# warlock-labs/sylow

Hardware: AMD Instinct MI355X
Metric: BN254 pairings/s (value) and BLS verifies/s (config.bls_verifies_per_s) at batch=2^20 per GPU (higher is better)
Workload: dtype i32/u32 limbs (9x29-bit carry-free core + 8x32-bit Montgomery, exact integer)

## Files before the change

sylow_amd/csrc/bn254_pair29.hpp:

```cpp
#pragma once
#include "bn254_f29.hpp"
#include "bn254_pair.hpp"

namespace bn254 {
namespace pl {

struct W2 { F29 c; };
BN_DEV const F29& f29_of(const W2& a) { return a.c; }
BN_DEV F29& f29_of(W2& a) { return a.c; }
struct W6 { W2 c0, c1, c2; };
struct W12 { W6 c0, c1; };

BN_DEV F29 xchg9(const F29& a) {
  F29 r;
#pragma unroll
  for (int i = 0; i < 9; ++i) r.v[i] = (i32)swap_u32((u32)a.v[i]);
  return r;
}
BN_DEV F29 sel9(bool odd, const F29& if_even, const F29& if_odd) {
  F29 r;
#pragma unroll
  for (int i = 0; i < 9; ++i) r.v[i] = odd ? if_odd.v[i] : if_even.v[i];
  return r;
}
// ... 174 lines not shown
  r.c1.c1 = w2_xi_lin(t2.v2, 1, w2_sub(w2_sub(t2.y1, t0.c1), t1.c1), 1);
  r.c1.c2 = w2_lin2(w2_sub(t2.y2, t0.c2), 1, t1.c2, -1);
}
BN_DEV W12 w12_mul(const W12& a, const W12& b) {
  const W6 t0 = w6_mul(a.c0, b.c0);
  const W6 t1 = w6_mul(a.c1, b.c1);
  const W6Raw t2 = w6_mul_raw(w6_add_norm(a.c0, a.c1), w6_add_norm(b.c0, b.c1));
  W12 r;
  w12_mul_c1(r, t2, t0, t1);
  r.c0.c0 = w2_xi_lin(t1.c2, 1, t0.c0, 1);
  r.c0.c1 = w2_norm(w2_add(t0.c1, t1.c0));
  r.c0.c2 = w2_norm(w2_add(t0.c2, t1.c1));
  return r;
}
BN_DEV W6 w6_mul_b2zero(const W6& a, const W6& b) {
  W2 v0, v1, p21, p20;
  W2_MUL2(v0, v1, a.c0, b.c0, a.c1, b.c1);
  W2_MUL2(p21, p20, a.c2, b.c1, a.c2, b.c0);
  const W2 s1 = w2_mul(w2_sub(a.c0, a.c1), w2_sub(b.c0, b.c1));
  W6 r;
  r.c0 = w2_xi_lin(p21, 1, v0, 1);
  r.c1 = w2_reduce(w2_sub(w2_add(v0, v1), s1));
  r.c2 = w2_norm(w2_add(p20, v1));
  return r;
}
BN_DEV W12 w12_mul_line_pair(const W12& a, const W12& b) {
  const W6 t0 = w6_mul(a.c0, b.c0);
  const W6 t1 = w6_mul_b2zero(a.c1, b.c1);
  const W6Raw t2 = w6_mul_raw(w6_add_norm(a.c0, a.c1), W6{w2_norm(w2_add(b.c0.c0, b.c1.c0)), w2_norm(w2_add(b.c0.c1, b.c1.c1)), b.c0.c2});
  W12 r;
  w12_mul_c1(r, t2, t0, t1);
  r.c0.c0 = w2_xi_lin(t1.c2, 1, t0.c0, 1);
  r.c0.c1 = w2_norm(w2_add(t0.c1, t1.c0));
  r.c0.c2 = w2_norm(w2_add(t0.c2, t1.c1));
  return r;
}
template <bool INL = false>
BN_DEV W12 w12_sqr(const W12& a) {
  const W6 d{w2_norm(w2_sub(a.c0.c0, a.c1.c0)), w2_norm(w2_sub(a.c0.c1, a.c1.c1)), w2_norm(w2_sub(a.c0.c2, a.c1.c2))};
  W6 e;
  e.c0 = w2_xi_lin(a.c1.c2, -1, a.c0.c0, 1);
  e.c1 = w2_norm(w2_sub(a.c0.c1, a.c1.c0));
  e.c2 = w2_norm(w2_sub(a.c0.c2, a.c1.c1));
  const W6 c2 = w6_mul<INL>(a.c0, a.c1);
  const W6Raw m = w6_mul_raw<INL>(d, e);
  W12 r;
  r.c1.c0 = w2_norm(w2_add(c2.c0, c2.c0));
  r.c1.c1 = w2_norm(w2_add(c2.c1, c2.c1));
  r.c1.c2 = w2_norm(w2_add(c2.c2, c2.c2));
  r.c0.c0 = w2_xi_lin(w2_add(m.x0, c2.c2), 1, w2_add(m.v0, c2.c0), 1);
  {
    const F29 xo = xchg9(m.v2.c);
    const W2 cc = w2_add(c2.c1, c2.c0);
    const F29* const t[4] = {&m.v2.c, &xo, &m.y1.c, &cc.c};
    const i32 c[4] = {bn_keep(9), bn_keep_v(lane_odd() ? 1 : -1), bn_keep(1), bn_keep(1)};
    r.c0.c1 = W2{f29_reduce_terms(t, c)};
  }
  r.c0.c2 = w2_lin2(m.y2, 1, w2_add(c2.c2, c2.c1), 1);
  return r;
}
BN_DEV W12 w12_conj(const W12& a) {
  W12 r;
  r.c0 = a.c0;
  r.c1.c0 = w2_norm(w2_neg(a.c1.c0)); r.c1.c1 = w2_norm(w2_neg(a.c1.c1)); r.c1.c2 = w2_norm(w2_neg(a.c1.c2));
  return r;
}
BN_DEV W2 w2_conj(const W2& a) { return W2{sel9(lane_odd(), a.c, f29_norm(f29_neg(a.c)))}; }
template <int E>
BN_DEV W6 w6_frobenius(const W6& a) {
  constexpr bool oddE = (E & 1) != 0;
  const uint32_t (&k1)[2][8] = (E == 1) ? C_FROB6_C1_1 : (E == 2) ? C_FROB6_C1_2 : C_FROB6_C1_3;
  const uint32_t (&k2)[2][8] = (E == 1) ? C_FROB6_C2_1 : (E == 2) ? C_FROB6_C2_2 : C_FROB6_C2_3;
  W6 r;
  r.c0 = oddE ? w2_conj(a.c0) : a.c0;
  W2_MUL2(r.c1, r.c2, oddE ? w2_conj(a.c1) : a.c1, w2_const(k1), oddE ? w2_conj(a.c2) : a.c2, w2_const(k2));
  return r;
}
template <int E>
BN_DEV W12 w12_frobenius(const W12& a) {
  const uint32_t (&k)[2][8] = (E == 1) ? C_FROB12_C1_1 : (E == 2) ? C_FROB12_C1_2 : C_FROB12_C1_3;
  const W2 kk = w2_const(k);
  const W6 x1 = w6_frobenius<E>(a.c1);
  W6 y;
  W2_MUL2(y.c0, y.c1, x1.c0, kk, x1.c1, kk);
  y.c2 = w2_mul(x1.c2, kk);
  return W12{w6_frobenius<E>(a.c0), y};
}
BN_DEV W12 w12_sparse_mul(const W12& f, const W2& x0, const W2& x4, const W2& x2) {
  const W2 z0 = f.c0.c0, z1 = f.c0.c1, z2 = f.c0.c2, z3 = f.c1.c0, z4 = f.c1.c1, z5 = f.c1.c2;
  W2 d0, d2, d4, p12, p54, p10, p34, p30, p52, q02, q24, q04;
  W2_MUL2(d0, d2, z0, x0, z2, x2);
  W2_MUL2(d4, p12, z4, x4, z1, x2);
  W2_MUL2(p54, p10, z5, x4, z1, x0);
  W2_MUL2(p34, p30, z3, x4, z3, x0);
  W2_MUL2(p52, q02, z5, x2, w2_sub(z0, z2), w2_sub(x0, x2));
  W2_MUL2(q24, q04, w2_sub(z2, z4), w2_sub(x2, x4), w2_sub(z0, z4), w2_sub(x0, x4));
  const W2 qs = w2_mul(w2_norm(w2_add(w2_add(z1, z3), z5)), w2_norm(w2_add(w2_add(x0, x2), x4)));
  W12 o;
  o.c0.c0 = w2_xi_lin(w2_add(p12, d4), 1, d0, 1);
  o.c0.c1 = w2_xi_lin(w2_add(p54, d2), 1, p10, 1);
  o.c0.c2 = w2_reduce(w2_add(w2_sub(w2_add(d0, d2), q02), p34));
  o.c1.c0 = w2_xi_lin(w2_sub(w2_add(d2, d4), q24), 1, p30, 1);
  o.c1.c1 = w2_xi_lin(p52, 1, w2_sub(w2_add(d0, d4), q04), 1);
  {
    const W2 sa = w2_add(w2_add(p12, p54), p10), sb = w2_add(w2_add(p34, p30), p52);
    const F29* const t[3] = {&qs.c, &sa.c, &sb.c};
    const i32 c[3] = {bn_keep(1), bn_keep(-1), bn_keep(-1)};
    o.c1.c2 = W2{f29_reduce_terms(t, c)};
  }
  return o;
}
BN_DEV W2 w2_xi_lin_v(const W2& x, const W2& y, i32 m) {
  const F29 xo = xchg9(x.c);
  const F29* const t[3] = {&x.c, &xo, &y.c};
  const i32 c[3] = {bn_keep(9), bn_keep_v(lane_odd() ? 1 : -1), bn_keep_v(m)};
  return W2{f29_reduce_terms(t, c)};
}
BN_DEV W2 w2_lin_v(const W2& x, const W2& y, i32 m) {
  const F29* const t[2] = {&x.c, &y.c};
  const i32 c[2] = {bn_keep(1), bn_keep_v(m)};
  return W2{f29_reduce_terms(t, c)};
}
BN_DEV W12 w12_sparse_mul_unit(const W12& f, i32 u, const W2& x4, const W2& x2) {
  const W2 z0 = f.c0.c0, z1 = f.c0.c1, z2 = f.c0.c2, z3 = f.c1.c0, z4 = f.c1.c1, z5 = f.c1.c2;
  W2 d2, d4, p12, p54, p34, p52, a02, a04, q24, q13;
  W2_MUL2(d2, d4, z2, x2, z4, x4);
  W2_MUL2(p12, p54, z1, x2, z5, x4);
  W2_MUL2(p34, p52, z3, x4, z5, x2);
  W2_MUL2(a02, a04, z0, x2, z0, x4);
  const W2 x24 = w2_sub(x2, x4);
  W2_MUL2(q24, q13, w2_sub(z2, z4), x24, w2_sub(z1, z3), x24);
  W12 o;
  o.c0.c0 = w2_xi_lin_v(w2_add(p12, d4), z0, u);
  o.c0.c1 = w2_xi_lin_v(w2_add(p54, d2), z1, u);
  o.c0.c2 = w2_lin_v(w2_add(a02, p34), z2, u);
  o.c1.c0 = w2_xi_lin_v(w2_sub(w2_add(d2, d4), q24), z3, u);
  {
    const F29 xo = xchg9(p52.c);
    const F29* const t[4] = {&p52.c, &xo, &a04.c, &z4.c};
    const i32 c[4] = {bn_keep(9), bn_keep_v(lane_odd() ? 1 : -1), bn_keep(1), bn_keep_v(u)};
    o.c1.c1 = W2{f29_reduce_terms(t, c)};
  }
  o.c1.c2 = w2_lin_v(w2_sub(w2_add(p12, p34), q13), z5, u);
  return o;
}
BN_DEV W2 w2_xi_norm(const W2& x, const W2& y) {
  const F29 xo = xchg9(x.c);
  const F29* const t[3] = {&x.c, &xo, &y.c};
  const i32 c[3] = {bn_keep(9), bn_keep_v(lane_odd() ? 1 : -1), bn_keep(1)};
  return W2{f29_norm_terms(t, c)};
}
BN_DEV W2 w2_xi_norm_sub(const W2& x, const W2& y) {
  const F29 xo = xchg9(x.c);
  const F29* const t[3] = {&x.c, &xo, &y.c};
  const i32 c[3] = {bn_keep(-9), bn_keep_v(lane_odd() ? -1 : 1), bn_keep(1)};
  return W2{f29_norm_terms(t, c)};
}
template <bool INL = false>
BN_DEV void w_fp4_square_fold(W2& out0, W2& m, const W2& a, const W2& b, const W2& z) {
  W2 w;
  W2_MUL2_SEL(INL, m, w, a, b, w2_sub(a, b), w2_xi_norm_sub(b, a));
  const F29 mo = xchg9(m.c);
  const F29* const t[4] = {&w.c, &m.c, &mo, &z.c};
  const i32 c[4] = {bn_keep(3), bn_keep(30), bn_keep_v(lane_odd() ? 3 : -3), bn_keep(-2)};
  out0 = W2{f29_reduce_terms(t, c)};
}
template <bool INL = false>
BN_DEV W12 w12_cyclotomic_sqr(const W12& f) {
  const W2 z0 = f.c0.c0, z4 = f.c0.c1, z3 = f.c0.c2, z2 = f.c1.c0, z1 = f.c1.c1, z5 = f.c1.c2;
  W2 m;
  W12 r;
  w_fp4_square_fold<INL>(r.c0.c0, m, z0, z1, z0);
  r.c1.c1 = w2_lin2(m, 6, z1, 2);
  w_fp4_square_fold<INL>(r.c0.c1, m, z2, z3, z4);
  r.c1.c2 = w2_lin2(m, 6, z5, 2);
  w_fp4_square_fold<INL>(r.c0.c2, m, z4, z5, z3);
  r.c1.c0 = w2_xi_lin(m, 6, z2, 2);
  return r;
}

BN_DEV F29 f29_halve(const F29& a) {
  i32 p[9]; f29_p(p);
  const i32 m = -(a.v[0] & 1);
  i32 lo[9];
  i32 c = 0;
#pragma unroll
  for (int i = 0; i < 8; ++i) {
    i32 t = a.v[i] + (p[i] & m) + c;
    lo[i] = t & BN_M29;
    c = t >> 29;
  }
  lo[8] = a.v[8] + (p[8] & m) + c;
  F29 r;
#pragma unroll
  for (int i = 0; i < 8; ++i) r.v[i] = (lo[i] >> 1) | ((lo[i + 1] & 1) << 28);
  r.v[8] = lo[8] >> 1;
  return r;
}
BN_DEV W2 w2_halve(const W2& a) { return W2{f29_halve(a.c)}; }
BN_DEV W2 w2_triple(const W2& a) { return W2{f29_add(f29_add(a.c, a.c), a.c)}; }
struct G2W { W2 x, y, z; };
BN_DEV W2 w2_twist_b() {
  const F29 k0{{0x12cb9911, 0x1fcb719e, 0x1368f727, 0x1ff96726, 0x0aadc75b, 0x179b4484, 0x06475c9b, 0x020e578d, -1520355}};
  const F29 k1{{0x0322ef99, 0x06e86c1b, 0x13f74e78, 0x0a0a4222, 0x0bcef269, 0x0af6e9ff, 0x0644c3a7, 0x0acd7c01, -535829}};
  return W2{sel9(lane_odd(), k0, k1)};
}
BN_DEV F29 f29_iso_s2() { return F29{{0x05beeef0, 0x1f76bf90, 0x1d5e46cf, 0x17f6764e, 0x1df385e5, 0x0d7a8334, 0x152215eb, 0x01b6eac1, -290196}}; }
BN_DEV F29 f29_iso_s3() { return F29{{0x1af1f8a3, 0x00cd9858, 0x1dce6a34, 0x142e620a, 0x1bc0c667, 0x0ae94d20, 0x0db9310b, 0x12572b72, 0x000405e6}}; }
BN_DEV W2 w2_mul_27m3u(const W2& a) {
  const F29 ao = xchg9(a.c);
  const F29* const t[2] = {&a.c, &ao};
  const i32 c[2] = {bn_keep(27), bn_keep_v(lane_odd() ? -3 : 3)};
  return W2{f29_reduce_terms(t, c)};
}
template <bool ISO = false>
BN_DEV void g2_doubling_step29(G2W& r, W2& l0, W2& l1, W2& l2) {
#if BN_QUAD
  W2 xy, xx, b, c, yz2, e;
  W2_MUL_SQR(xy, xx, r.x, r.y, r.x);
  const W2 a = w2_halve(xy);
  l2 = w2_norm(w2_triple(xx));
  W2_SQR2(b, c, r.y, r.z);
  if (ISO) {
    yz2 = w2_sqr(w2_norm(w2_add(r.y, r.z)));
    e = w2_mul_27m3u(c);
  } else {
    W2_SQR_MUL(yz2, e, w2_norm(w2_add(r.y, r.z)), w2_twist_b(), w2_norm(w2_triple(c)));
  }
  const W2 h = w2_norm(w2_sub(yz2, w2_add(b, c)));
  l1 = w2_neg(h);
  l0 = w2_xi_lin(w2_sub(e, b), 1, b, 0);
  const W2 f = w2_norm(w2_triple(e));
  W2_MUL2(r.z, r.x, b, h, a, w2_sub(b, f));
  const W2 g = w2_halve(w2_norm(w2_add(b, f)));
  W2 gg, ee;
  W2_SQR2(gg, ee, g, e);
  r.y = w2_lin2(gg, 1, ee, -3);
#else
  const W2 a = w2_halve(w2_mul(r.x, r.y));
  l2 = w2_norm(w2_triple(w2_sqr(r.x)));
  const W2 b = w2_sqr(r.y);
  const W2 c = w2_sqr(r.z);
  const W2 h = w2_norm(w2_sub(w2_sqr(w2_norm(w2_add(r.y, r.z))), w2_add(b, c)));
  const W2 e = ISO ? w2_mul_27m3u(c) : w2_mul(w2_twist_b(), w2_norm(w2_triple(c)));
  l1 = w2_neg(h);
  r.z = w2_mul(b, h);
  l0 = w2_xi_lin(w2_sub(e, b), 1, b, 0);
  const W2 f = w2_norm(w2_triple(e));
  r.x = w2_mul(a, w2_sub(b, f));
  const W2 g = w2_halve(w2_norm(w2_add(b, f)));
  r.y = w2_lin2(w2_sqr(g), 1, w2_sqr(e), -3);
#endif
}
BN_DEV void g2_addition_step29(G2W& r, const W2& bx, const W2& by, W2& l0, W2& l1, W2& l2) {
#if BN_QUAD
  W2 zbx, zby, ebx, dby;
  W2_MUL2(zbx, zby, r.z, bx, r.z, by);
  const W2 d = w2_sub(r.x, zbx);
  const W2 e = w2_sub(r.y, zby);
  W2_MUL2(ebx, dby, e, bx, d, by);
  l0 = w2_xi_lin(w2_sub(ebx, dby), 1, bx, 0);
  l1 = d;
  l2 = w2_neg(e);
  const W2 dn = w2_norm(d), en = w2_norm(e);
  W2 f, ee, h, i, zee, zh, dj, hy;
  W2_SQR2(f, ee, dn, en);
  W2_MUL2(h, i, dn, f, r.x, f);
  W2_MUL2(zee, zh, r.z, ee, r.z, h);
  const W2 j = w2_norm(w2_sub(w2_add(zee, h), w2_add(i, i)));
  W2_MUL2(dj, hy, dn, j, h, r.y);
  r.z = zh;
  r.x = dj;
  r.y = w2_norm(w2_sub(w2_mul(en, w2_sub(i, j)), hy));
#else
  const W2 d = w2_sub(r.x, w2_mul(r.z, bx));
  const W2 e = w2_sub(r.y, w2_mul(r.z, by));
  l0 = w2_xi_lin(w2_sub(w2_mul(e, bx), w2_mul(d, by)), 1, bx, 0);
  l1 = d;
  l2 = w2_neg(e);
  const W2 dn = w2_norm(d), en = w2_norm(e);
  const W2 f = w2_sqr(dn);
  const W2 h = w2_mul(dn, f);
  const W2 i = w2_mul(r.x, f);
  const W2 j = w2_norm(w2_sub(w2_add(w2_mul(r.z, w2_sqr(en)), h), w2_add(i, i)));
  r.z = w2_mul(r.z, h);
  r.x = w2_mul(dn, j);
  r.y = w2_norm(w2_sub(w2_mul(en, w2_sub(i, j)), w2_mul(h, r.y)));
#endif
}
BN_DEV W12 w12_line_product(const W2& a0, const W2& a4, const W2& a2, const W2& b0, const W2& b4, const W2& b2) {
  W2 d0, d2, d4, k02, k24, k04;
  W2_MUL2(d0, d2, a0, b0, a2, b2);
  W2_MUL2(d4, k02, a4, b4, w2_sub(a0, a2), w2_sub(b0, b2));
  W2_MUL2(k24, k04, w2_sub(a2, a4), w2_sub(b2, b4), w2_sub(a0, a4), w2_sub(b0, b4));
  W12 r;
  r.c0.c0 = w2_xi_lin(d4, 1, d0, 1);
  r.c0.c1 = w2_xi_lin(d2, 1, d2, 0);
  r.c0.c2 = w2_reduce(w2_sub(w2_add(d0, d2), k02));
  r.c1.c0 = w2_xi_lin(w2_sub(w2_add(d2, d4), k24), 1, d2, 0);
  r.c1.c1 = w2_reduce(w2_sub(w2_add(d0, d4), k04));
  r.c1.c2 = W2{F29{{0, 0, 0, 0, 0, 0, 0, 0, 0}}};
  return r;
}
constexpr int MILLER_LDS_WORDS = 36, MILLER_LDS_WORDS_PARK = 63;
BN_DEV void lds_put9(i32 (*lds)[256], int slot, const F29& a) {
#pragma unroll
  for (int i = 0; i < 9; ++i) lds[9 * slot + i][threadIdx.x] = a.v[i];
}
BN_DEV F29 lds_get9(i32 (*lds)[256], int slot) {
  F29 r;
#pragma unroll
  for (int i = 0; i < 9; ++i) r.v[i] = lds[9 * slot + i][threadIdx.x];
  return r;
}
#ifndef BN_MILLER_SQR_INL
#define BN_MILLER_SQR_INL false
#endif
template <bool PARK, bool ISO = false>
BN_NOINLINE void miller_loop29g(S12& fout, const Fp& pxs, const Fp& pys, const S2& qxs_in, const S2& qys_in) {
  __shared__ i32 lds[PARK ? MILLER_LDS_WORDS_PARK : MILLER_LDS_WORDS][256];
  S2 qxs = qxs_in, qys = qys_in;
  {
    const F29 px = f29_reduce(f29_from_fp(pxs)), py = f29_reduce(f29_from_fp(pys));
    lds_put9(lds, 0, ISO ? f29_mul(px, f29_iso_s2()) : px);
    lds_put9(lds, 1, ISO ? f29_mul(py, f29_iso_s3()) : py);
  }
  {
    W2 qx = w2_from_s2(qxs), qy = w2_from_s2(qys);
    if (ISO) {
      W2_SCALE2(qx, qy, qx, f29_iso_s2(), qy, f29_iso_s3());
      qxs = w2_to_s2(qx); qys = w2_to_s2(qy);
    }
    lds_put9(lds, 2, qx.c);
    lds_put9(lds, 3, qy.c);
  }
  auto PX = [&]() { return lds_get9(lds, 0); };
  auto PY = [&]() { return lds_get9(lds, 1); };
  auto QX = [&]() { return W2{lds_get9(lds, 2)}; };
  auto QY = [&](bool neg) { const W2 y{lds_get9(lds, 3)}; return neg ? w2_neg(y) : y; };
  auto park = [&](const G2W& r) { if (PARK) { lds_put9(lds, 4, r.x.c); lds_put9(lds, 5, r.y.c); lds_put9(lds, 6, r.z.c); } };
  auto unpark = [&](const G2W& r) { return PARK ? G2W{W2{lds_get9(lds, 4)}, W2{lds_get9(lds, 5)}, W2{lds_get9(lds, 6)}} : r; };
  W12 f;
  G2W r{QX(), QY(false), w2_from_s2(s2_one())};
  W2 l0, l1, l2;
  auto line_mul = [&](const W12& x) {
    W2 s1, s2;
    W2_SCALE2(s1, s2, l1, PY(), l2, PX());
    return w12_sparse_mul(x, l0, s1, s2);
  };
  const u64 nz = BN_ATE_NAF_NZ, ng = BN_ATE_NAF_NEG;
  static_assert((BN_ATE_NAF_NZ >> 63) & 1, "the first digit of 6x+2 after the leading one is non-zero");
  {
    g2_doubling_step29<ISO>(r, l0, l1, l2);
    const W2 d0 = l0;
    W2 d4, d2, e4, e2;
    W2_SCALE2(d4, d2, l1, PY(), l2, PX());
    g2_addition_step29(r, QX(), QY((ng >> 63) & 1), l0, l1, l2);
    park(r);
    W2_SCALE2(e4, e2, l1, PY(), l2, PX());
    f = w12_line_product(d0, d4, d2, l0, e4, e2);
  }
#pragma unroll 1
  for (int i = 1; i < 64; ++i) {
    r = unpark(r);
    g2_doubling_step29<ISO>(r, l0, l1, l2);
    park(r);
    f = w12_sqr<BN_MILLER_SQR_INL>(f);
    f = line_mul(f);
    if ((nz >> (63 - i)) & 1) {
      r = unpark(r);
      g2_addition_step29(r, QX(), QY((ng >> (63 - i)) & 1), l0, l1, l2);
      park(r);
      f = line_mul(f);
    }
  }
  r = unpark(r);
  S2 q1x, q1y, q2x, q2y;
  g2_psi_affine(q1x, q1y, qxs, qys);
  g2_psi_affine(q2x, q2y, q1x, q1y);
  q2y = s2_neg(q2y);
  g2_addition_step29(r, w2_from_s2(q1x), w2_from_s2(q1y), l0, l1, l2);
  f = line_mul(f);
  g2_addition_step29(r, w2_from_s2(q2x), w2_from_s2(q2y), l0, l1, l2);
  f = line_mul(f);
  w12_to_s12(fout, f);
}


BN_DEV void w12_pin(W12& x) {
  W2* const c[6] = {&x.c0.c0, &x.c0.c1, &x.c0.c2, &x.c1.c0, &x.c1.c1, &x.c1.c2};
#pragma unroll
  for (int j = 0; j < 6; ++j)
#pragma unroll
    for (int i = 0; i < 9; ++i) BN_CHAIN_NV(c[j]->c.v[i]);
}
BN_NOINLINE void w12_mul_nl(W12& r, const W12& a, const W12& b) {
  W12 x = a, y = b;
  w12_pin(x); w12_pin(y);
  r = w12_mul(x, y);
}
BN_NOINLINE void w12_cyclotomic_sqr_nl(W12& r, const W12& a) {
  W12 x = a;
  w12_pin(x);
  r = w12_cyclotomic_sqr(x);
}
template <int E> BN_NOINLINE void w12_frobenius_nl(W12& r, const W12& a) {
  W12 x = a;
  w12_pin(x);
  r = w12_frobenius<E>(x);
}
#ifndef BN_EXP_INL
#define BN_EXP_INL true
#endif
#define BN_X_C_NZ 0x0008144402208421ull
#define BN_X_C_NEG 0x0008004400000020ull
#define BN_X_C_17 0x0000100000008021ull
BN_NOINLINE void exp_by_neg_z29(W12& r, const W12& f) {
  W12 tab[2];
  {
    W12 t, u;
    w12_cyclotomic_sqr_nl(t, f);
    w12_cyclotomic_sqr_nl(u, t);
    w12_cyclotomic_sqr_nl(t, u);
    w12_cyclotomic_sqr_nl(u, t);
    w12_mul_nl(tab[0], u, f);
    w12_cyclotomic_sqr_nl(t, tab[0]);
    w12_mul_nl(tab[1], t, f);
  }
  W12 res = tab[1];
  const u64 nz = BN_X_C_NZ, ng = BN_X_C_NEG, i17 = BN_X_C_17;
#pragma unroll 1
  for (int i = 56; i >= 0; --i) {
    res = w12_cyclotomic_sqr<BN_EXP_INL>(res);
    if ((nz >> i) & 1) {
      W12 m = tab[((i17 >> i) & 1) ? 0 : 1];
      if ((ng >> i) & 1) m = w12_conj(m);
      res = w12_mul(res, m);
    }
  }
  r = w12_conj(res);
}
BN_DEV W2 w2_inv(const W2& a) {
  const F29 t = f29_mul_leaf(W_ARGS(a.c), W_ARGS(a.c));
  const F29 n = f29_norm(f29_add(t, xchg9(t)));
  const F29 i = f29_reduce(f29_from_fp(fp_inv(f29_to_fp(n))));
  const F29 r = f29_mul_leaf(W_ARGS(a.c), W_ARGS(i));
  return W2{sel9(lane_odd(), r, f29_norm(f29_neg(r)))};
}
BN_DEV W2 w2_mul_xi(const W2& a) { return w2_xi_lin(a, 1, a, 0); }
BN_DEV W6 w6_inv(const W6& a) {
  W2 s0, m12, s2, m01, s1, m02, u1, u2, o0, o1;
  W2_SQR_MUL(s0, m12, a.c0, a.c1, w2_mul_xi(a.c2));
  W2_SQR_MUL(s2, m01, a.c2, a.c0, a.c1);
  W2_SQR_MUL(s1, m02, a.c1, a.c0, a.c2);
  const W2 t0 = w2_sub(s0, m12);
  const W2 t1 = w2_sub(w2_mul_xi(s2), m01);
  const W2 t2 = w2_sub(s1, m02);
  W2_MUL2(u1, u2, a.c2, t1, a.c1, t2);
  const W2 d = w2_xi_lin(w2_add(u1, u2), 1, w2_mul(a.c0, t0), 1);
  const W2 di = w2_inv(d);
  W2_MUL2(o0, o1, di, t0, di, t1);
  return W6{o0, o1, w2_mul(di, t2)};
}
BN_NOINLINE void w12_inv_nl(W12& r, const W12& ain) {
  W12 a = ain;
  w12_pin(a);
  const W6 s0 = w6_mul(a.c0, a.c0), s1 = w6_mul(a.c1, a.c1);
  const W6 d{w2_norm(w2_sub(s0.c0, w2_mul_xi(s1.c2))), w2_norm(w2_sub(s0.c1, s1.c0)), w2_norm(w2_sub(s0.c2, s1.c1))};
  const W6 t = w6_inv(d);
  r.c0 = w6_mul(a.c0, t);
  const W6 m = w6_mul(a.c1, t);
  r.c1 = W6{w2_norm(w2_neg(m.c0)), w2_norm(w2_neg(m.c1)), w2_norm(w2_neg(m.c2))};
}
BN_NOINLINE void final_exponentiation29(S12& out, const S12& fin) {
  W12 in, t, a, b, d, e, g;
  {
    w12_from_s12(t, fin);
    w12_inv_nl(b, t);
    a = w12_conj(t);
    w12_mul_nl(d, a, b);
    w12_frobenius_nl<2>(a, d);
    w12_mul_nl(in, a, d);
  }
  exp_by_neg_z29(a, in);
  w12_cyclotomic_sqr_nl(b, a);
  w12_cyclotomic_sqr_nl(t, b);
  w12_mul_nl(d, t, b);
  exp_by_neg_z29(e, d);
  w12_cyclotomic_sqr_nl(t, e);
  exp_by_neg_z29(g, t);
  d = w12_conj(d);
  g = w12_conj(g);
  w12_mul_nl(t, g, e);
  w12_mul_nl(a, t, d);
  w12_mul_nl(d, a, b);
  w12_mul_nl(t, a, e);
  w12_mul_nl(e, in, t);
  w12_frobenius_nl<1>(t, d);
  w12_mul_nl(b, t, e);
  w12_frobenius_nl<2>(t, a);
  w12_mul_nl(e, t, b);
  t = w12_conj(in);
  w12_mul_nl(a, t, d);
  w12_frobenius_nl<3>(t, a);
  w12_mul_nl(g, t, e);
  w12_to_s12(out, g);
}


#ifdef BN_WIDE_LEAF_CALL
BN_DEV W2 w2_mul_w(const W2& a, const W2& b) { return w2_mul(a, b); }
#else
BN_DEV W2 w2_mul_w(const W2& a, const W2& b) { return w2_mul_inl(a, b); }
#endif
struct alignas(16) WideLds { i32 v[63][2][12]; };
typedef __attribute__((address_space(3))) WideLds* WideLdsPtr;
template <int EPW> BN_DEV int wide_j(int lane) { return (int)pair_index((u32)lane) & (32 / EPW - 1); }
typedef i32 __attribute__((ext_vector_type(4))) WideVec4;
typedef __attribute__((address_space(3))) WideVec4* WideVec4Ptr;
BN_DEV void wide_put(WideLdsPtr x, int slot, int odd, const W2& a) {
  const WideVec4Ptr p = (WideVec4Ptr)&x->v[slot][odd][0];
  p[0] = WideVec4{a.c.v[0], a.c.v[1], a.c.v[2], a.c.v[3]};
  p[1] = WideVec4{a.c.v[4], a.c.v[5], a.c.v[6], a.c.v[7]};
  x->v[slot][odd][8] = a.c.v[8];
}
BN_DEV W2 wide_get(WideLdsPtr x, int slot, int odd) {
  const WideVec4Ptr p = (WideVec4Ptr)&x->v[slot][odd][0];
  const WideVec4 lo = p[0], hi = p[1];
  W2 r;
  r.c.v[0] = lo.x; r.c.v[1] = lo.y; r.c.v[2] = lo.z; r.c.v[3] = lo.w;
  r.c.v[4] = hi.x; r.c.v[5] = hi.y; r.c.v[6] = hi.z; r.c.v[7] = hi.w;
  r.c.v[8] = x->v[slot][odd][8];
  return r;
}
BN_DEV W2 w2_pick(const W2& a, const W2& b, bool c) { return W2{sel9(c, a.c, b.c)}; }
BN_DEV W2 w2_real(const F29& k) { return W2{sel9(lane_odd(), k, F29{{0, 0, 0, 0, 0, 0, 0, 0, 0}})}; }
BN_DEV W2 w2_sel3(int k, const W2& a, const W2& b, const W2& c) { return w2_pick(w2_pick(a, b, k == 1), c, k == 2); }
template <int EPW = 1>
BN_DEV W12 w12_cyclotomic_sqr_wide(const W12& f, WideLdsPtr x) {
  const int lane = (int)(threadIdx.x & 63u), odd = pair_role((u32)lane), j = wide_j<EPW>(lane);
  const int p = j < 6 ? j : 0, k = p >> 1;
  const bool s = (p & 1) != 0;
  const W2 z0 = f.c0.c0, z4 = f.c0.c1, z3 = f.c0.c2, z2 = f.c1.c0, z1 = f.c1.c1, z5 = f.c1.c2;
  const W2 a = w2_sel3(k, z0, z2, z4), b = w2_sel3(k, z1, z3, z5);
  {
    const W2 xs = w2_pick(a, w2_norm(w2_add(a, b)), s), ys = w2_pick(b, w2_xi_norm(b, a), s);
    const W2 pr = w2_mul_w(xs, ys);
    if (j < 6) wide_put(x, p, odd, pr);
  }
  __syncthreads();
  {
    const int ko = p < 2 ? 0 : p < 4 ? 2 : 1;
    const bool ta = p == 0 || p == 3 || p == 4, tc = p == 2;
    const W2 m = wide_get(x, 2 * ko, odd), w = wide_get(x, 2 * ko + 1, odd);
    const W2 z = w2_pick(a, b, s);
    const F29 mo = xchg9(m.c);
    const bool lo = lane_odd();
    const F29* const t[4] = {&w.c, &m.c, &mo, &z.c};
    const i32 c[4] = {bn_keep_v(ta ? 3 : 0), bn_keep_v(ta ? -30 : tc ? 54 : 6), bn_keep_v(ta ? (lo ? -3 : 3) : tc ? (lo ? 6 : -6) : 0), bn_keep_v(ta ? -2 : 2)};
    const W2 r{f29_reduce_terms(t, c)};
    if (j < 6) wide_put(x, 6 + (p < 2 ? p : p < 4 ? p + 2 : p - 2), odd, r);
  }
  __syncthreads();
  W12 r;
  r.c0.c0 = wide_get(x, 6, odd); r.c1.c1 = wide_get(x, 7, odd); r.c0.c1 = wide_get(x, 8, odd);
  r.c1.c2 = wide_get(x, 9, odd); r.c1.c0 = wide_get(x, 10, odd); r.c0.c2 = wide_get(x, 11, odd);
  return r;
}
constexpr int WL_IA = 12, WL_IB = 18, WL_SA = 24, WL_SB = 27, WL_P = 30, WL_T = 48, WL_OUT = 57;
constexpr int WK_DENSE = 0, WK_LINE = 1, WK_SQUARE = 2;
#ifndef BN_WIDE_MILLER_INL
#define BN_WIDE_MILLER_INL 2
#endif
#ifndef BN_WIDE_KINDS
#define BN_WIDE_KINDS 1
#endif
BN_DEV W2 w12_coef(const W12& a, int c) {
  const W2 lo = w2_sel3(c % 3, a.c0.c0, a.c0.c1, a.c0.c2), hi = w2_sel3(c % 3, a.c1.c0, a.c1.c1, a.c1.c2);
  return w2_pick(lo, hi, c >= 3);
}
template <int EPW = 1, int KIND = WK_DENSE>
BN_DEV void w12_mul_wide_stage0(const W12& a, const W12& b, WideLdsPtr x) {
  const int lane = (int)(threadIdx.x & 63u), odd = pair_role((u32)lane), j = wide_j<EPW>(lane);
  {
    const int c = j < 6 ? j : 0;
    const int i = c % 3;
    const W2 a0i = w2_sel3(i, a.c0.c0, a.c0.c1, a.c0.c2), a1i = w2_sel3(i, a.c1.c0, a.c1.c1, a.c1.c2);
    const W2 sa = w2_norm(w2_add(a0i, a1i));
    if (KIND == WK_SQUARE) {
      const W2 sb0 = w2_xi_lin(a.c1.c2, 1, a.c0.c0, 1);
      const W2 sb12 = w2_norm(w2_add(a0i, w2_pick(a.c1.c0, a.c1.c1, i == 2)));
      if (j < 3) { wide_put(x, WL_IA + i, odd, a0i); wide_put(x, WL_IB + i, odd, a1i); wide_put(x, WL_SA + i, odd, sa); }
      if (j >= 3 && j < 6) wide_put(x, WL_SB + i, odd, w2_pick(sb12, sb0, i == 0));
    } else {
      const W2 ac = w2_pick(a0i, a1i, c >= 3), bc = w12_coef(b, c);
      const W2 sb = w2_norm(w2_add(w2_sel3(i, b.c0.c0, b.c0.c1, b.c0.c2), w2_sel3(i, b.c1.c0, b.c1.c1, b.c1.c2)));
      if (j < 6) { wide_put(x, WL_IA + c, odd, ac); wide_put(x, WL_IB + c, odd, bc); }
      if (j < 3) wide_put(x, WL_SA + i, odd, sa);
      if (j >= 3 && j < 6) wide_put(x, WL_SB + i, odd, sb);
    }
  }
}
template <int EPW = 1, int KIND = WK_DENSE, bool STAGE3 = true>
BN_DEV void w12_mul_wide_core(WideLdsPtr x) {
  const int lane = (int)(threadIdx.x & 63u), odd = pair_role((u32)lane), j = wide_j<EPW>(lane);
  const W2 zero{F29{{0, 0, 0, 0, 0, 0, 0, 0, 0}}};
  __syncthreads();
#pragma unroll
  for (int pass = 0; pass < (KIND == WK_DENSE ? EPW : 1); ++pass) {
    int w;
    bool live;
    if (KIND == WK_DENSE) {
      const int jw = j + 16 * pass;
      live = jw < 18;
      w = live ? jw : 0;
    } else if (KIND == WK_LINE) {
      live = j < 14;
      w = live ? j + (j >= 1) + (j >= 5) + (j >= 6) + (j >= 8) : 0;
    } else {
      live = j < 12;
      w = j < 6 ? j : live ? j + 6 : 0;
    }
    const int g = w / 6, h = w % 6;
    const int i0 = h < 3 ? h : h == 3 ? 1 : 0, i1 = h < 3 ? h : h == 4 ? 1 : 2;
    const int ba = g == 0 ? WL_IA : g == 1 ? WL_IA + 3 : WL_SA, bb = g == 0 ? WL_IB : g == 1 ? WL_IB + 3 : WL_SB;
    const W2 xa = wide_get(x, ba + i0, odd), xb = wide_get(x, ba + i1, odd);
    const W2 ya = wide_get(x, bb + i0, odd), yb = wide_get(x, bb + i1, odd);
    const W2 xs = w2_pick(xa, w2_norm(w2_add(xa, xb)), h >= 3), ys = w2_pick(ya, w2_norm(w2_add(ya, yb)), h >= 3);
    const W2 pr = w2_mul_w(xs, ys);
    if (live) wide_put(x, WL_P + w, odd, pr);
    if (KIND == WK_LINE && j < 4) wide_put(x, WL_P + (int)((0x0B080601u >> (8 * j)) & 255u), odd, zero);
  }
  __syncthreads();
  {
    const int nu = KIND == WK_SQUARE ? 6 : 9;
    const int u = j >= nu ? 0 : (KIND == WK_SQUARE && j >= 3) ? j + 3 : j, g = u / 3, c = u % 3, base = WL_P + 6 * g;
    const W2 v0 = wide_get(x, base, odd), v1 = wide_get(x, base + 1, odd), v2 = wide_get(x, base + 2, odd), q = wide_get(x, base + 3 + c, odd);
    const W2 xv = w2_pick(v2, w2_sub(w2_sub(q, v1), v2), c == 0);
    const F29 xo = xchg9(xv.c);
    const bool lo = lane_odd();
    const F29* const t[6] = {&xv.c, &xo, &q.c, &v0.c, &v1.c, &v2.c};
    const i32 kx = c == 2 ? 0 : 1;
    const i32 k[6] = {bn_keep_v(9 * kx), bn_keep_v(lo ? kx : -kx), bn_keep_v(c == 0 ? 0 : 1), bn_keep_v(c == 0 ? 1 : -1),
                      bn_keep_v(c == 0 ? 0 : c == 1 ? -1 : 1), bn_keep_v(c == 2 ? -1 : 0)};
    if (j < nu) wide_put(x, WL_T + u, odd, W2{f29_reduce_terms(t, k)});
  }
  __syncthreads();
  if (!STAGE3) return;
  if (KIND == WK_SQUARE) {
    const int o = j < 6 ? j : 0, i = o % 3;
    const W2 ti = wide_get(x, WL_T + i, odd), tp = wide_get(x, WL_T + (i + 2) % 3, odd), mi = wide_get(x, WL_T + 6 + i, odd);
    const F29 tpo = xchg9(tp.c);
    const bool lo = lane_odd(), hi = o >= 3, o0 = o == 0;
    const F29* const t[4] = {&ti.c, &tp.c, &tpo, &mi.c};
    const i32 k[4] = {bn_keep_v(hi ? 2 : -1), bn_keep_v(hi ? 0 : o0 ? -9 : -1), bn_keep_v(o0 ? (lo ? -1 : 1) : 0), bn_keep_v(hi ? 0 : 1)};
    if (j < 6) wide_put(x, WL_OUT + o, odd, W2{f29_reduce_terms(t, k)});
  } else {
    const int o = j < 6 ? j : 0, i = o % 3;
    const int pa = o >= 3 ? i : o, pb = o >= 3 ? 3 + i : o == 0 ? 5 : o == 1 ? 3 : 4, pc = o >= 3 ? 6 + i : 0;
    const W2 ta = wide_get(x, WL_T + pa, odd), tb = wide_get(x, WL_T + pb, odd), tc = wide_get(x, WL_T + pc, odd);
    const F29 tbo = xchg9(tb.c);
    const bool lo = lane_odd(), hi = o >= 3, o0 = o == 0;
    const F29* const t[4] = {&ta.c, &tb.c, &tbo, &tc.c};
    const i32 k[4] = {bn_keep_v(hi ? -1 : 1), bn_keep_v(hi ? -1 : o0 ? 9 : 1), bn_keep_v(o0 ? (lo ? 1 : -1) : 0), bn_keep_v(hi ? 1 : 0)};
    if (j < 6) wide_put(x, WL_OUT + o, odd, W2{f29_reduce_terms(t, k)});
  }
  __syncthreads();
}
BN_DEV W12 w12_wide_result(WideLdsPtr x) {
  const int odd = pair_role((u32)(threadIdx.x & 63u));
  W12 r;
  r.c0.c0 = wide_get(x, WL_OUT, odd); r.c0.c1 = wide_get(x, WL_OUT + 1, odd); r.c0.c2 = wide_get(x, WL_OUT + 2, odd);
  r.c1.c0 = wide_get(x, WL_OUT + 3, odd); r.c1.c1 = wide_get(x, WL_OUT + 4, odd); r.c1.c2 = wide_get(x, WL_OUT + 5, odd);
  return r;
}
template <int EPW = 1, int KIND = WK_DENSE>
BN_DEV W12 w12_mul_wide(const W12& a, const W12& b, WideLdsPtr x) {
  w12_mul_wide_stage0<EPW, KIND>(a, b, x);
  w12_mul_wide_core<EPW, KIND>(x);
  return w12_wide_result(x);
}
template <int EPW = 1, int KIND = WK_DENSE>
BN_NOINLINE void w12_mul_wide_core_nl(WideLds* xg) { w12_mul_wide_core<EPW, KIND>((WideLdsPtr)xg); }
template <int EPW = 1, int KIND = WK_DENSE>
BN_DEV void w12_mul_wide_nl(W12& r, const W12& a, const W12& b, WideLds* xg) {
  w12_mul_wide_stage0<EPW, KIND>(a, b, (WideLdsPtr)xg);
  w12_mul_wide_core_nl<EPW, KIND>(xg);
  r = w12_wide_result((WideLdsPtr)xg);
}
template <int EPW = 1>
BN_NOINLINE void exp_by_neg_z29_wide(W12& r, const W12& f, WideLds* xg) {
  const WideLdsPtr x = (WideLdsPtr)xg;
  W12 tab[2];
  {
    W12 t = f;
#pragma unroll 1
    for (int k = 0; k < 5; ++k) {
      t = w12_cyclotomic_sqr_wide<EPW>(t, x);
      if (k == 3) {
        w12_mul_wide_nl<EPW>(tab[0], t, f, xg);
        t = tab[0];
      }
    }
    w12_mul_wide_nl<EPW>(tab[1], t, f, xg);
  }
  W12 res = tab[1];
  const u64 nz = BN_X_C_NZ, ng = BN_X_C_NEG, i17 = BN_X_C_17;
#pragma unroll 1
  for (int i = 56; i >= 0; --i) {
    res = w12_cyclotomic_sqr_wide<EPW>(res, x);
    if ((nz >> i) & 1) {
      W12 m = tab[((i17 >> i) & 1) ? 0 : 1];
      if ((ng >> i) & 1) m = w12_conj(m);
      res = w12_mul_wide<EPW>(res, m, x);
    }
  }
  r = w12_conj(res);
}
template <int E, int EPW = 1>
BN_DEV W12 w12_frobenius_wide(const W12& a, WideLdsPtr x) {
  constexpr bool oddE = (E & 1) != 0;
  const int lane = (int)(threadIdx.x & 63u), odd = pair_role((u32)lane), j = wide_j<EPW>(lane);
  const W2 k1 = w2_const((E == 1) ? C_FROB6_C1_1 : (E == 2) ? C_FROB6_C1_2 : C_FROB6_C1_3);
  const W2 k2 = w2_const((E == 1) ? C_FROB6_C2_1 : (E == 2) ? C_FROB6_C2_2 : C_FROB6_C2_3);
  const W2 kk = w2_const((E == 1) ? C_FROB12_C1_1 : (E == 2) ? C_FROB12_C1_2 : C_FROB12_C1_3);
  {
    const int p = j < 5 ? j : 0;
    const W2 c = w2_pick(w2_pick(w2_pick(w2_pick(a.c0.c1, a.c0.c2, p == 1), a.c1.c0, p == 2), a.c1.c1, p == 3), a.c1.c2, p == 4);
    const W2 u = oddE ? w2_conj(c) : c;
    const W2 v = w2_pick(w2_pick(k1, k2, p == 1 || p == 4), kk, p == 2);
    const W2 pr = w2_mul_w(u, v);
    if (j < 5) wide_put(x, WL_P + p, odd, pr);
  }
  __syncthreads();
  {
    const W2 u = wide_get(x, WL_P + 3 + (j == 1 ? 1 : 0), odd);
    const W2 pr = w2_mul_w(u, kk);
    if (j < 2) wide_put(x, WL_T + j, odd, pr);
  }
  __syncthreads();
  W12 r;
  r.c0.c0 = oddE ? w2_conj(a.c0.c0) : a.c0.c0;
  r.c0.c1 = wide_get(x, WL_P, odd); r.c0.c2 = wide_get(x, WL_P + 1, odd);
  r.c1.c0 = wide_get(x, WL_P + 2, odd); r.c1.c1 = wide_get(x, WL_T, odd); r.c1.c2 = wide_get(x, WL_T + 1, odd);
  return r;
}
template <int EPW>
BN_DEV void w6_mul2_wide(const W6& a, const W6& b, const W6& c, const W6& d, WideLdsPtr x) {
  const int lane = (int)(threadIdx.x & 63u), odd = pair_role((u32)lane), j = wide_j<EPW>(lane);
  const int i = (j < 6 ? j : 0) % 3;
  const bool hi = j >= 3;
  const W2 u = w2_sel3(i, w2_pick(a.c0, c.c0, hi), w2_pick(a.c1, c.c1, hi), w2_pick(a.c2, c.c2, hi));
  const W2 v = w2_sel3(i, w2_pick(b.c0, d.c0, hi), w2_pick(b.c1, d.c1, hi), w2_pick(b.c2, d.c2, hi));
  if (j < 3) { wide_put(x, WL_IA + i, odd, u); wide_put(x, WL_IB + i, odd, v); }
  if (j >= 3 && j < 6) { wide_put(x, WL_SA + i, odd, u); wide_put(x, WL_SB + i, odd, v); }
  w12_mul_wide_core<EPW, WK_SQUARE, false>(x);
}
BN_DEV W6 w6_wide_t(WideLdsPtr x, int base) {
  const int odd = pair_role((u32)(threadIdx.x & 63u));
  return W6{wide_get(x, WL_T + base, odd), wide_get(x, WL_T + base + 1, odd), wide_get(x, WL_T + base + 2, odd)};
}
template <int EPW = 1>
BN_DEV W12 w12_inv_wide(const W12& a, WideLdsPtr x) {
  const int lane = (int)(threadIdx.x & 63u), odd = pair_role((u32)lane), j = wide_j<EPW>(lane);
  w6_mul2_wide<EPW>(a.c0, a.c0, a.c1, a.c1, x);
  const W6 s0 = w6_wide_t(x, 0), s1 = w6_wide_t(x, 6);
  const W2 d0 = w2_norm(w2_sub(s0.c0, w2_mul_xi(s1.c2))), d1 = w2_norm(w2_sub(s0.c1, s1.c0)), d2 = w2_norm(w2_sub(s0.c2, s1.c1));
  {
    const int p = j < 6 ? j : 0;
    const W2 xd2 = w2_mul_xi(d2);
    const W2 u = w2_pick(w2_pick(d0, d1, p == 1 || p == 4), d2, p == 2);
    const W2 v = w2_pick(w2_pick(w2_pick(w2_pick(d0, xd2, p == 1), d2, p == 2 || p == 5), d1, p == 3 || p == 4), d0, p == 0);
    const W2 pr = w2_mul_w(u, v);
    if (j < 6) wide_put(x, WL_P + p, odd, pr);
  }
  __syncthreads();
  const W2 t0 = w2_sub(wide_get(x, WL_P, odd), wide_get(x, WL_P + 1, odd));
  const W2 t1 = w2_sub(w2_mul_xi(wide_get(x, WL_P + 2, odd)), wide_get(x, WL_P + 3, odd));
  const W2 t2 = w2_sub(wide_get(x, WL_P + 4, odd), wide_get(x, WL_P + 5, odd));
  {
    const int p = j < 3 ? j : 0;
    const W2 pr = w2_mul_w(w2_sel3(p, d2, d1, d0), w2_sel3(p, t1, t2, t0));
    if (j < 3) wide_put(x, WL_P + 6 + p, odd, pr);
  }
  __syncthreads();
  const W2 dd = w2_xi_lin(w2_add(wide_get(x, WL_P + 6, odd), wide_get(x, WL_P + 7, odd)), 1, wide_get(x, WL_P + 8, odd), 1);
  const W2 di = w2_inv(dd);
  {
    const int p = j < 3 ? j : 0;
    const W2 pr = w2_mul_w(di, w2_sel3(p, t0, t1, t2));
    if (j < 3) wide_put(x, WL_P + 9 + p, odd, pr);
  }
  __syncthreads();
  const W6 t{wide_get(x, WL_P + 9, odd), wide_get(x, WL_P + 10, odd), wide_get(x, WL_P + 11, odd)};
  w6_mul2_wide<EPW>(a.c0, t, a.c1, t, x);
  const W6 m = w6_wide_t(x, 6);
  W12 r;
  r.c0 = w6_wide_t(x, 0);
  r.c1 = W6{w2_norm(w2_neg(m.c0)), w2_norm(w2_neg(m.c1)), w2_norm(w2_neg(m.c2))};
  return r;
}
template <int EPW = 1>
BN_NOINLINE void final_exponentiation29_wide(S12& out, const S12& fin, WideLds* x) {
  W12 in, t, a, b, d, e, g;
  {
    w12_from_s12(t, fin);
    b = w12_inv_wide<EPW>(t, (WideLdsPtr)x);
    a = w12_conj(t);
    w12_mul_wide_nl<EPW>(d, a, b, x);
// ... 157 lines not shown
```

sylow_amd/csrc/plk_verify_body.hpp:

```cpp
#pragma once
#include "plk_common.hpp"

namespace plk {
BN_DEV void stage_table(i32* lds, const i32* src) {
  for (int k = threadIdx.x; k < LINE_TABLE_WORDS; k += blockDim.x) lds[k] = src[k];
}
BN_DEV W2 table_w2(const i32* tab, int at, int c, int odd) {
  const i32* t = tab + ((at * 2 + c) * 2 + odd) * 9;
  return W2{F29{{t[0], t[1], t[2], t[3], t[4], t[5], t[6], t[7], t[8]}}};
}
BN_DEV i32 table_unit(const i32* tab, int at) { return tab[LINE_TABLE_LINES * 36 + at]; }

template <bool PK_TABLE>
BN_DEV void bls_verify_fused_body(const u64* pkxy, const uint8_t* pkinf, const i32* pk_table,
                                  const u64* hneg, const uint8_t* hneg_inf,
                                  const u64* sigxy, const uint8_t* siginf, const i32* gen_table, uint8_t* okout, size_t n, size_t m, const Stagger& st) {
  __shared__ i32 tabA[LINE_TABLE_WORDS];
  __shared__ i32 tabB[PK_TABLE ? LINE_TABLE_WORDS : 1];
  unsigned chunk;
  int role = stagger_role(st, chunk);
  const size_t t = (size_t)chunk * blockDim.x + threadIdx.x, i = elem_index(t);
  const int odd = pair_role(t);
  const size_t np = (size_t)st.count * ELEMS_PER_BLOCK, ip = (size_t)(chunk - st.first) * ELEMS_PER_BLOCK + (i & (ELEMS_PER_BLOCK - 1));
  if (role == 2 && !stagger_wait(st, chunk)) role = 0;
  if (role == 2) {
    S12 fs, g;
    load_s12(fs, st.park, np, ip, odd);
    final_exponentiation29(g, fs);
    const bool one = s12_is_one(g);
    if (!odd && elem_writer(t)) okout[i] = one ? 1 : 0;
    return;
  }
  stage_table(tabA, gen_table);
  if (PK_TABLE) stage_table(tabB, pk_table);
  __syncthreads();
  const bool active = i < m;
  const size_t ii = active ? i : 0;
  const Fp hxs = load_fp(hneg, n, ii, 0), hys = load_fp(hneg, n, ii, 4);
  const bool hinf = hneg_inf[ii] != 0;
  __shared__ i32 lds[PK_TABLE ? 36 : 54][256];
  const bool liveA = !(siginf && siginf[ii]);
  const bool liveB = !(hinf || (pkinf && pkinf[PK_TABLE ? 0 : ii]));
  const F29 f29_zero{{0, 0, 0, 0, 0, 0, 0, 0, 0}};
  lds_put9(lds, 0, liveA ? f29_reduce(f29_from_fp(load_fp(sigxy, n, ii, 0))) : f29_zero);
  lds_put9(lds, 1, liveA ? f29_reduce(f29_from_fp(load_fp(sigxy, n, ii, 4))) : f29_zero);
  constexpr bool ISO = !PK_TABLE;
  lds_put9(lds, 2, liveB ? (ISO ? f29_mul(f29_reduce(f29_from_fp(hxs)), f29_iso_s2()) : f29_reduce(f29_from_fp(hxs))) : f29_zero);
  lds_put9(lds, 3, liveB ? (ISO ? f29_mul(f29_reduce(f29_from_fp(hys)), f29_iso_s3()) : f29_reduce(f29_from_fp(hys))) : f29_zero);
  auto SX = [&]() { return lds_get9(lds, 0); };
  auto SY = [&]() { return lds_get9(lds, 1); };
  auto HX = [&]() { return lds_get9(lds, 2); };
  auto HY = [&]() { return lds_get9(lds, 3); };
  auto key_x = [&]() { return (PK_TABLE || !liveB) ? s2_g2gen_x() : load_s2(pkxy, n, ii, 0, odd); };
  auto key_y = [&]() { return (PK_TABLE || !liveB) ? s2_g2gen_y() : load_s2(pkxy, n, ii, 8, odd); };
  G2W r;
  {
    W2 qx = w2_from_s2(key_x()), qy = w2_from_s2(key_y());
    if (ISO) W2_SCALE2(qx, qy, qx, f29_iso_s2(), qy, f29_iso_s3());
    if (!PK_TABLE) { lds_put9(lds, 4, qx.c); lds_put9(lds, 5, qy.c); }
    r = G2W{qx, qy, w2_from_s2(s2_one())};
  }
  auto QX = [&]() { return W2{lds_get9(lds, PK_TABLE ? 0 : 4)}; };
  auto QY = [&](bool neg) {
    const W2 y{lds_get9(lds, PK_TABLE ? 0 : 5)};
    return neg ? w2_neg(y) : y;
  };
  W12 f;
  {
    S12 one = s12_one();
    w12_from_s12(f, one);
  }
  W2 l0, l1, l2;
  int idx = 0;
  auto lineA = [&]() {
    W2 a1, a2;
    W2_SCALE2(a1, a2, table_w2(tabA, idx, 0, odd), SY(), table_w2(tabA, idx, 1, odd), SX());
    f = w12_sparse_mul_unit(f, liveA ? table_unit(tabA, idx) : 1, a1, a2);
  };
  auto lineB = [&]() {
    if (PK_TABLE) {
      W2 b1, b2;
      W2_SCALE2(b1, b2, table_w2(tabB, idx, 0, odd), HY(), table_w2(tabB, idx, 1, odd), HX());
      f = w12_sparse_mul_unit(f, liveB ? table_unit(tabB, idx) : 1, b1, b2);
    } else {
      W2 s1, s2;
      W2_SCALE2(s1, s2, l1, HY(), l2, HX());
      f = w12_sparse_mul(f, l0, s1, s2);
    }
  };
  const u64 nz = BN_ATE_NAF_NZ, ng = BN_ATE_NAF_NEG;
#pragma unroll 1
  for (int it = 0; it < 64; ++it) {
    f = w12_sqr(f);
    lineA();
    if (!PK_TABLE) g2_doubling_step29<ISO>(r, l0, l1, l2);
    lineB();
    ++idx;
    if ((nz >> (63 - it)) & 1) {
      lineA();
      if (!PK_TABLE) g2_addition_step29(r, QX(), QY(((ng >> (63 - it)) & 1) != 0), l0, l1, l2);
      lineB();
      ++idx;
    }
  }
  S2 q1x, q1y, q2x, q2y;
  if (!PK_TABLE) { g2_psi_affine(q1x, q1y, w2_to_s2(QX()), w2_to_s2(QY(false))); g2_psi_affine(q2x, q2y, q1x, q1y); }
  lineA();
  if (!PK_TABLE) g2_addition_step29(r, w2_from_s2(q1x), w2_from_s2(q1y), l0, l1, l2);
  lineB();
  ++idx;
  lineA();
  if (!PK_TABLE) g2_addition_step29(r, w2_from_s2(q2x), w2_from_s2(s2_neg(q2y)), l0, l1, l2);
  lineB();
  S12 fs, g;
  w12_to_s12(fs, f);
  if (role == 1) {
    store_s12(st.park, np, ip, odd, fs);
    stagger_publish(st, chunk);
    return;
  }
  final_exponentiation29(g, fs);
  const bool one = s12_is_one(g);
  if (active && !odd && elem_writer(t)) okout[i] = one ? 1 : 0;
}
}
```

Measured before the change: 9.731 million.

## Peel first Miller iteration and skip last final-exp multiply via equality test

```diff
diff --git a/sylow_amd/csrc/bn254_pair29.hpp b/sylow_amd/csrc/bn254_pair29.hpp
--- a/sylow_amd/csrc/bn254_pair29.hpp
+++ b/sylow_amd/csrc/bn254_pair29.hpp
@@ -500,6 +500,20 @@
   r.c1.c2 = W2{F29{{0, 0, 0, 0, 0, 0, 0, 0, 0}}};
   return r;
 }
+BN_DEV W12 w12_unit_line_product(i32 u, const W2& a4, const W2& a2, i32 t, const W2& b4, const W2& b2, const W2& one) {
+  W2 d2, d4;
+  W2_MUL2(d2, d4, a2, b2, a4, b4);
+  const W2 k24 = w2_mul(w2_sub(a2, a4), w2_sub(b2, b4));
+  W12 r;
+  r.c0.c0 = w2_xi_lin_v(d4, one, u * t);
+  r.c0.c1 = w2_xi_lin(d2, 1, d2, 0);
+  r.c1.c0 = w2_xi_lin(w2_sub(w2_add(d2, d4), k24), 1, d2, 0);
+  const F29 zero{{0, 0, 0, 0, 0, 0, 0, 0, 0}};
+  r.c0.c2 = w2_lin_v(W2{sel9(u != 0, zero, b2.c)}, a2, t);
+  r.c1.c1 = w2_lin_v(W2{sel9(u != 0, zero, b4.c)}, a4, t);
+  r.c1.c2 = W2{F29{{0, 0, 0, 0, 0, 0, 0, 0, 0}}};
+  return r;
+}
 constexpr int MILLER_LDS_WORDS = 36, MILLER_LDS_WORDS_PARK = 63;
 BN_DEV void lds_put9(i32 (*lds)[256], int slot, const F29& a) {
 #pragma unroll
@@ -670,8 +684,8 @@
   const W6 m = w6_mul(a.c1, t);
   r.c1 = W6{w2_norm(w2_neg(m.c0)), w2_norm(w2_neg(m.c1)), w2_norm(w2_neg(m.c2))};
 }
-BN_NOINLINE void final_exponentiation29(S12& out, const S12& fin) {
-  W12 in, t, a, b, d, e, g;
+BN_DEV void final_exponentiation29_factors(W12& t, W12& e, const S12& fin) {
+  W12 in, a, b, d, g;
   {
     w12_from_s12(t, fin);
     w12_inv_nl(b, t);
@@ -701,8 +715,25 @@
   t = w12_conj(in);
   w12_mul_nl(a, t, d);
   w12_frobenius_nl<3>(t, a);
+}
+BN_NOINLINE void final_exponentiation29(S12& out, const S12& fin) {
+  W12 t, e, g;
+  final_exponentiation29_factors(t, e, fin);
   w12_mul_nl(g, t, e);
   w12_to_s12(out, g);
+}
+BN_NOINLINE bool final_exponentiation29_is_one(const S12& fin) {
+  W12 t, e;
+  final_exponentiation29_factors(t, e, fin);
+  const bool fin_zero = s2_is_zero(fin.c0.c0) && s2_is_zero(fin.c0.c1) && s2_is_zero(fin.c0.c2) &&
+                        s2_is_zero(fin.c1.c0) && s2_is_zero(fin.c1.c1) && s2_is_zero(fin.c1.c2);
+  bool z = s2_is_zero(w2_to_s2(w2_norm(w2_sub(t.c0.c0, e.c0.c0))));
+  z = s2_is_zero(w2_to_s2(w2_norm(w2_sub(t.c0.c1, e.c0.c1)))) && z;
+  z = s2_is_zero(w2_to_s2(w2_norm(w2_sub(t.c0.c2, e.c0.c2)))) && z;
+  z = s2_is_zero(w2_to_s2(w2_norm(w2_add(t.c1.c0, e.c1.c0)))) && z;
+  z = s2_is_zero(w2_to_s2(w2_norm(w2_add(t.c1.c1, e.c1.c1)))) && z;
+  z = s2_is_zero(w2_to_s2(w2_norm(w2_add(t.c1.c2, e.c1.c2)))) && z;
+  return z && !fin_zero;
 }
 
 
diff --git a/sylow_amd/csrc/plk_verify_body.hpp b/sylow_amd/csrc/plk_verify_body.hpp
--- a/sylow_amd/csrc/plk_verify_body.hpp
+++ b/sylow_amd/csrc/plk_verify_body.hpp
@@ -24,10 +24,9 @@
   const size_t np = (size_t)st.count * ELEMS_PER_BLOCK, ip = (size_t)(chunk - st.first) * ELEMS_PER_BLOCK + (i & (ELEMS_PER_BLOCK - 1));
   if (role == 2 && !stagger_wait(st, chunk)) role = 0;
   if (role == 2) {
-    S12 fs, g;
+    S12 fs;
     load_s12(fs, st.park, np, ip, odd);
-    final_exponentiation29(g, fs);
-    const bool one = s12_is_one(g);
+    const bool one = final_exponentiation29_is_one(fs);
     if (!odd && elem_writer(t)) okout[i] = one ? 1 : 0;
     return;
   }
@@ -66,10 +65,6 @@
     return neg ? w2_neg(y) : y;
   };
   W12 f;
-  {
-    S12 one = s12_one();
-    w12_from_s12(f, one);
-  }
   W2 l0, l1, l2;
   int idx = 0;
   auto lineA = [&]() {
@@ -89,8 +84,32 @@
     }
   };
   const u64 nz = BN_ATE_NAF_NZ, ng = BN_ATE_NAF_NEG;
+  static_assert((BN_ATE_NAF_NZ >> 63) & 1, "the first digit of 6x+2 after the leading one is non-zero");
+  {
+    const W2 one = w2_from_s2(s2_one());
+    auto unit_pair = [&](const i32* tab, bool live, const F29& py, const F29& px) {
+      W2 a4, a2, b4, b2;
+      W2_SCALE2(a4, a2, table_w2(tab, 0, 0, odd), py, table_w2(tab, 0, 1, odd), px);
+      W2_SCALE2(b4, b2, table_w2(tab, 1, 0, odd), py, table_w2(tab, 1, 1, odd), px);
+      return w12_unit_line_product(live ? table_unit(tab, 0) : 1, a4, a2, live ? table_unit(tab, 1) : 1, b4, b2, one);
+    };
+    W12 fb;
+    if (PK_TABLE) {
+      fb = unit_pair(tabB, liveB, HY(), HX());
+    } else {
+      g2_doubling_step29<ISO>(r, l0, l1, l2);
+      const W2 d0 = l0;
+      W2 d4, d2, e4, e2;
+      W2_SCALE2(d4, d2, l1, HY(), l2, HX());
+      g2_addition_step29(r, QX(), QY(((ng >> 63) & 1) != 0), l0, l1, l2);
+      W2_SCALE2(e4, e2, l1, HY(), l2, HX());
+      fb = w12_line_product(d0, d4, d2, l0, e4, e2);
+    }
+    f = w12_mul_line_pair(fb, unit_pair(tabA, liveA, SY(), SX()));
+    idx = 2;
+  }
 #pragma unroll 1
-  for (int it = 0; it < 64; ++it) {
+  for (int it = 1; it < 64; ++it) {
     f = w12_sqr(f);
     lineA();
     if (!PK_TABLE) g2_doubling_step29<ISO>(r, l0, l1, l2);
@@ -112,15 +131,14 @@
   lineA();
   if (!PK_TABLE) g2_addition_step29(r, w2_from_s2(q2x), w2_from_s2(s2_neg(q2y)), l0, l1, l2);
   lineB();
-  S12 fs, g;
+  S12 fs;
   w12_to_s12(fs, f);
   if (role == 1) {
     store_s12(st.park, np, ip, odd, fs);
     stagger_publish(st, chunk);
     return;
   }
-  final_exponentiation29(g, fs);
-  const bool one = s12_is_one(g);
+  const bool one = final_exponentiation29_is_one(fs);
   if (active && !odd && elem_writer(t)) okout[i] = one ? 1 : 0;
 }
 }
```

Result: no change. 9.731 million, median of 2 (-0.0%).
